# stulacy/bmm-mcmc

Hardware: AMD Instinct MI355X
Metric: gibbs_sweeps_per_s (higher is better)
Workload: dtype f64; 1 GPU; c5: gibbs_collapsed K=20 N=10000000 P=100, 1 chain per GPU; sampler=collapsed, K=20, N=10000000, P=100, batch=2500000, chains=1, chains_per_gpu=1, burn_sweeps=30, x_layout=bit planes, ceil(P/32) words per observation, packed once at hand-over

## Files before the change

bmm-mcmc_amd/csrc/chain.hip:

```cpp
#include <hip/hip_runtime.h>
#include <hip/hip_ext.h>
#include <rccl/rccl.h>

#include <dlfcn.h>
#include <emmintrin.h>
#include <sched.h>
#include <sys/mman.h>

#include <cmath>
#include <cstdarg>
#include <cstdio>
#include <cstdint>
#include <cstdlib>
#include <cstring>
#include <atomic>
#include <chrono>
#include <condition_variable>
#include <exception>
#include <functional>
#include <limits>
#include <memory>
#include <mutex>
#include <new>
#include <string>
// ... 267 lines not shown
#ifndef BMM_SMALL_SPLIT
#define BMM_SMALL_SPLIT 1
#endif
#ifndef BMM_SELF_TABLES
#define BMM_SELF_TABLES 1
#endif
constexpr int kStageWide = BMM_STAGE_WIDE;

constexpr int threads_for(int kt, bool bits) {
    if (bits) return kt <= 20 ? kThreadsSmall : (kt <= 32 ? kThreadsMid : kThreadsLarge);
    return kt <= 12 ? kThreadsSmall : (kt <= 20 ? kThreadsMid : kThreadsLarge);
}

struct KernelForm {
    int kt = 0;
    int nt = 0;
    int minus = 0;
    bool bits = false;
    int lanes = 1;
    bool emit = false;
    int gw = kGroupW;
    bool self = false;
    bool pk = false;
};
constexpr int tile_of(const KernelForm& f) { return f.nt / f.lanes; }
constexpr KernelForm resized(KernelForm f, int nt, int lanes = 1) { f.nt = nt; f.lanes = lanes; return f; }
constexpr KernelForm emit_twin(const KernelForm& f) {
    return KernelForm{f.kt, threads_for(f.kt, true), f.minus, true, 1, true, f.gw, false};
}

constexpr int stage_width(const KernelForm& f, bool named_size) {
    if (f.bits || f.kt > 20 || f.nt == 256) return 16;
    if (f.nt == kThreadsSmall) return f.nt == threads_for(f.kt, false) && !named_size ? kStageWide : 16;
    return kStageWide;
}

constexpr bool instantiated(const KernelForm& f, bool named_size) {
    const bool preferred = f.gw == kGroupW;
    if (f.pk) return f.bits && f.lanes == 1 && f.minus == 1 && !f.emit && !f.self && f.kt <= 32 &&
                     (preferred || (f.gw == kGroupWAlt && f.nt == threads_for(f.kt, true)));
    if (f.self) return f.kt <= 12 && f.nt == 256 && f.minus == 1 && f.bits && f.lanes == 1 && !f.emit && preferred;
    if (f.emit) return f.bits && f.lanes == 1 && f.nt == threads_for(f.kt, true);
    if (f.lanes == 2) return f.bits && f.nt == kThreadsSplit && f.minus != 2 && (f.kt > 32 || (f.kt >= 16 && preferred));
    if (f.lanes != 1) return false;
    if (f.nt == threads_for(f.kt, f.bits) && !named_size) return true;
    if (!preferred || f.minus == 2) return false;
    if (f.nt == 256) return true;
    return (f.nt == 1024 || f.nt == 768 || f.nt == 512) && f.kt <= 32 && (f.bits || f.minus == 1);
}

typedef void (*resample_fn)(ChainParams, ResampleArgs);
template <int KT, int NT, int MINUS, bool BITS, int GW, int LANES, bool EMIT, bool SELF, bool NAMED>
resample_fn instance() {
    constexpr KernelForm F{KT, NT, MINUS, BITS, LANES, EMIT, GW, SELF};
    if constexpr (instantiated(F, NAMED)) return k_resample<KT, NT, MINUS, stage_width(F, NAMED), BITS, LANES, EMIT, GW, SELF>;
    else return nullptr;
}
resample_fn lookup(const KernelForm& f, bool named_size = false) {
    resample_fn fn = nullptr;
    if (f.pk) {
        if (!instantiated(f, named_size)) return nullptr;
        lift([&](auto kt, auto nt, auto gw) {
            if constexpr (instantiated(KernelForm{kt, nt, 1, true, 1, false, gw, false, true}, false)) fn = k_resample_pk<kt, nt, gw>;
        }, kKT, f.kt, IntList<1024, 768, 512, 256>{}, f.nt, IntList<kGroupW, kGroupWAlt>{}, f.gw);
        return fn;
    }
    lift([&](auto kt, auto nt, auto minus, auto bits, auto gw) {
        if (f.lanes == 2) fn = f.emit || f.self ? nullptr : instance<kt, nt, minus, bits != 0, gw, 2, false, false, false>();
        else if (f.lanes != 1 || (f.emit && f.self)) fn = nullptr;
        else if (f.emit) fn = instance<kt, nt, minus, bits != 0, gw, 1, true, false, false>();
        else if (f.self) fn = instance<kt, nt, minus, bits != 0, gw, 1, false, true, false>();
        else if (named_size) fn = instance<kt, nt, minus, bits != 0, gw, 1, false, false, true>();
        else fn = instance<kt, nt, minus, bits != 0, gw, 1, false, false, false>();
    }, kKT, f.kt, IntList<1024, 768, 512, 256>{}, f.nt, IntList<0, 1, 2>{}, f.minus, IntList<0, 1>{}, (int)f.bits,
       IntList<kGroupW, kGroupWAlt>{}, f.gw);
    return fn;
}

constexpr int kLooMaxOwnKT = 32;
typedef void (*score_fn)(ChainParams, ScoreArgs);
score_fn lookup_score(int kt, int gw, int minus, bool loo) {
    score_fn fn = nullptr;
    lift([&](auto KT, auto GW, auto MINUS) {
        if constexpr (MINUS == 0) fn = loo ? k_score<KT, kScoreThreads, GW, 0, true> : k_score<KT, kScoreThreads, GW, 0, false>;
        else if constexpr (KT <= kLooMaxOwnKT) fn = loo ? k_score<KT, kScoreThreads, GW, MINUS, true> : nullptr;
    }, kKT, kt, IntList<kGroupW, kGroupWAlt>{}, gw, IntList<0, 1, 2>{}, minus);
// ... 283 lines not shown

constexpr int64_t kLargeN = (int64_t)1 << 16;
int64_t default_batch(int sampler, int64_t N) {
    if (sampler == BMM_SAMPLER_SB || sampler == BMM_SAMPLER_FULL) return N;
    const int64_t div = N >= kLargeN ? 4 : (sampler == BMM_SAMPLER_DP ? 16 : 8);
    const int64_t b = N / div;
    return b < 1 ? 1 : b;
}

TableLayout layout_of(const bmm_chain* c) { return layout_of(c->p, !explicit_params(c->p.mode)); }

int dbg_env_int(const char* name, int unset) { const char* v = dbg_env(name); return v ? (atoi(v) > 0 ? atoi(v) : 0) : unset; }
struct DebugSwitches {
    bool generic = dbg_env("BMM_DEBUG_GENERIC");
    bool int32_layout = dbg_env("BMM_X_LAYOUT_INT32");
    int cus = dbg_env_int("BMM_DEBUG_CUS", 0);
    int threads = dbg_env_int("BMM_DEBUG_THREADS", -1);
    bool split = dbg_env("BMM_DEBUG_SPLIT");
    bool nosplit = dbg_env("BMM_DEBUG_NOSPLIT");
    bool small = dbg_env("BMM_DEBUG_SMALL");
    bool noself = dbg_env("BMM_DEBUG_NOSELF");
    bool nopk = dbg_env("BMM_DEBUG_NOPK");
    bool pk = dbg_env("BMM_DEBUG_PK");
    int pk_defer_every = dbg_env_int("BMM_DEBUG_PK_DEFER_EVERY", 0);
};

struct ChainShape {
    ChainParams p{};
    int64_t batch = 1;
    bool generic = false;
    int minus_in_lds = 1;
    size_t lds_bytes_base = 0;
};
ChainParams geometry(int sampler, int P, int K, int kt, int W) {
    ChainParams q{};
    q.mode = sampler; q.P = P; q.K = K; q.KT = kt; q.W = W;
    q.G = (P + W - 1) / W; q.Gm = (P + kGroupWm - 1) / kGroupWm;
    q.Kc = sampler == BMM_SAMPLER_DP ? K + 1 : K;
    return q;
}
size_t image_bytes(const ChainParams& q, bool own_tables) {
    const TableLayout l = layout_of(q, own_tables && !explicit_params(q.mode));
    return (size_t)(own_tables ? l.doubles() : l.head()) * sizeof(double) + ((size_t)q.K * q.P + q.K + 4) * sizeof(int32_t);
}

size_t pk_image_bytes(const ChainParams& q) {
// ... 141 lines not shown
        const size_t off = (used + 255) & ~(size_t)255;
        used = off + n * sizeof(T);
        return base ? reinterpret_cast<T*>(base + off) : nullptr;
    }
};

int chain_alloc(bmm_chain* c) {
    const ChainParams& p = c->p;
    HIP_TRY(hipSetDevice(c->device));
    {
        int rcs = chain_stream_create(c, false);
        if (rcs) return rcs;
    }
    const size_t nz = (size_t)p.N;
    const size_t ns = (size_t)p.K * p.P, nn = (size_t)p.K;
    const size_t ntab = (size_t)layout_of(c).doubles() + (explicit_params(p.mode) ? 0 : 2 * (size_t)pk_tq_doubles(layout_of(c)));
    auto carve = [&](Carver& a) {
        c->dNk = a.take<int32_t>(nn);
        c->dDNk = a.take<int32_t>(nn * kDeltaReps);
        c->dS = a.take<int32_t>(ns);
        c->dDS = a.take<int32_t>(ns * kDeltaReps);
        c->dTab = a.take<double>(ntab);
#ifdef BMM_DIAG
        c->dDiag = a.take<unsigned long long>(16);
#endif
        c->dSelfDone = a.take<int>(1);
        c->dViable = a.take<int>(1);
        c->dDNkAlt = a.take<int32_t>(nn * kDeltaReps);
        c->dDSAlt = a.take<int32_t>(ns * kDeltaReps);
#ifdef BMM_DEBUG_HOOKS
        c->dDbgFlag = a.take<int>(1);
        c->dPkStat = a.take<unsigned long long>(3);
#endif
        const size_t zeroed = a.used;
        c->dAlpha = a.take<double>(1);
        c->dPi = a.take<double>(nn);
        c->dTheta = a.take<double>(ns);
        c->dZ[0] = a.take<int32_t>(nz);
        c->dZ[1] = a.take<int32_t>(nz);
        return zeroed;
    };
    Carver measure{nullptr};
    carve(measure);
    c->arena = static_cast<char*>(dev_pool().get(c->device, measure.used, &c->arena_bytes));
    if (!c->arena) return set_err(BMM_E_HIP, "allocating the chain's state failed: %s", hipGetErrorString(hipGetLastError()));
    Carver real{c->arena};
    const size_t zeroed = carve(real);
// ... 635 lines not shown
    if (c->fs_on) {
        const int rc = enqueue_fs_gamma(c, j);
        if (rc) return rc;
    }
    const int rc = sweep_end_folds(c, j);
    return rc == BMM_OK && c->na_on ? enqueue_na_step(c, j) : rc;
}

struct KernelPlan {
    int n = 0;
    KernelForm form[3];
    size_t lds[3] = {0, 0, 0};
    bool named_size = false;
};
KernelPlan plan_kernel(const ChainParams& p, bool bits, int minus, int64_t batch, int num_cus, bool shares_device,
                       size_t lds_bytes_base, const DebugSwitches& d, bool masked = false) {
    const bool alt = p.W != kGroupW;
    KernelForm f{p.KT, threads_for(p.KT, bits), minus, bits, 1, false, p.W, false};
    KernelPlan plan;
    const size_t pk_lds = explicit_params(p.mode) ? 0 : pk_image_bytes(p);
    auto offer = [&](KernelForm g, size_t lds) {
        KernelForm h = g;
        h.pk = true;
#ifdef BMM_EXP_PK_ALWAYS
        const bool long_launch = true;
#else
        const bool long_launch = batch >= (int64_t)4 * num_cus * g.nt;
#endif
        if (!masked && !d.nopk && (long_launch || d.pk) && !g.self && !explicit_params(p.mode) && instantiated(h, false) &&
            pk_lds <= kLdsMax && batch < ((int64_t)1 << 31)) { g = h; lds = pk_lds; }
        plan.form[plan.n] = g; plan.lds[plan.n++] = lds;
    };
    const bool short_launch = BMM_SMALL_SPLIT && !shares_device && p.KT >= 16 && !alt && (batch < (int64_t)num_cus * kThreadsMid || d.split);
    if (bits && (p.KT > 32 || short_launch) && minus != 2 && !d.nosplit) {
        const KernelForm g = resized(f, kThreadsSplit, 2);
        if (instantiated(g, false)) f = g;
    }
    if (d.threads >= 0 && !alt) {
        const KernelForm g = resized(f, d.threads);
        if (instantiated(g, true) && (p.KT <= 20 || (bits && g.nt != 1024))) { f = g; plan.named_size = true; }
    } else if (bits && f.lanes == 1 && !alt) {
        for (int nt : {768, 512}) {
            if ((batch + f.nt - 1) / f.nt >= num_cus || nt >= f.nt || (batch + nt - 1) / nt > num_cus) continue;
            if (instantiated(resized(f, nt), false)) f = resized(f, nt);
        }
    }
// ... 186 lines not shown
    c->minus_in_lds = shape.minus_in_lds;
    c->lds_bytes_base = c->lds_bytes = shape.lds_bytes_base;
    if (c->generic) {
        c->form = KernelForm{p.KT, 256, tier_of(c), c->bits, 1, false, p.W, false};
        c->scratch_stride = generic_threads(p.Kc);
        c->grid_max = (int)(c->scratch_stride / 256);
    } else {
        c->num_cus = dbg.cus >= 1 ? dbg.cus : cus;
        rc = pick_kernel(c);
        if (rc) { delete c; return rc; }
    }
    rc = chain_alloc(c);
    if (rc) { bmm_chain_destroy(c); return rc; }
    *out = c;
    return BMM_OK;
}

void bmm_chain_destroy(bmm_chain* c) {
    if (!c) return;
    (void)hipSetDevice(c->device);
    if (c->stream) (void)hipStreamSynchronize(c->stream);
#ifdef BMM_DIAG
    if (c->dDiag) {
        unsigned long long d[16] = {};
        const bool ok = hipMemcpy(d, c->dDiag, sizeof d, hipMemcpyDeviceToHost) == hipSuccess;
        if (ok && d[5] && d[0]) {
            const double tot = (double)(d[0] + d[1] + d[2] + d[3] + d[4]);
            fprintf(stderr, "[bmm diag] waves=%llu cycles/wave: score %.0f (%.1f%%) pack %.0f (%.1f%%) draw %.0f (%.1f%%) movers %.0f (%.1f%%) prologue %.0f (%.1f%%) movers/wave-launch %.2f\n",
                    d[5], d[0] / (double)d[5], 100 * d[0] / tot, d[1] / (double)d[5], 100 * d[1] / tot, d[2] / (double)d[5],
                    100 * d[2] / tot, d[3] / (double)d[5], 100 * d[3] / tot, d[4] / (double)d[5], 100 * d[4] / tot, d[6] / (double)d[5]);
        }
        if (ok && d[5])
            fprintf(stderr, "[bmm diag launch] ticks per wave and launch: table staging %.0f, tile loop %.0f, waiting for the workgroup %.0f, flush %.0f\n",
                    d[8] / (double)d[5], d[9] / (double)d[5], d[10] / (double)d[5], d[11] / (double)d[5]);
        if (ok && d[7])
            fprintf(stderr, "[bmm diag launch pk] workgroup-launches %llu, ticks from entry to flushed %.0f\n", d[7], d[14] / (double)d[7]);
        if (ok && d[5] && d[12])
            fprintf(stderr, "[bmm diag draw] draws of a wave (64 observations) %llu, of them by the binary64 definition %llu (%.4f%%)\n",
                    d[12], d[13], 100.0 * (double)d[13] / (double)d[12]);
    }
#endif
    for (hipEvent_t e : c->ev) (void)hipEventDestroy(e);
    if (c->planes && c->planes->refs.fetch_sub(1) == 1) {
        dev_pool().put(c->device, c->planes->d, c->planes->bytes);
        delete c->planes;
    }
    dev_pool().put(c->device, c->arena, c->arena_bytes);
    dev_pool().put(c->device, c->run_arena, c->run_arena_bytes);
    void* bufs[] = {c->dX_owned, c->dScratch, c->dProbs, c->dWts, c->dWtot, c->dXnb, c->dPredTab, c->dPredMax, c->dPredSum, c->dRespAcc,
                    c->dLooTab, c->dLooAcc, c->dLooOut, c->dLooScratch, c->dSmSide, c->dSmSideLaunch, c->dSmLq, c->dSmStat, c->dSmCell,
                    c->dSmCounters, c->dFsBlock, c->dEaBlock, c->dEaSide, c->dAsBlock, c->dLjBlock, c->dLjZ, c->dPcFeat, c->dPcXt, c->dPcBlock, c->dNaBlock};
    for (void* b : bufs)
        if (b) (void)hipFree(b);
    chain_stream_release(c->device, c->stream, c->stream_kind);
    delete c;
}

static int pack_rows(bmm_chain* c, const int32_t* dX, int64_t rows, int64_t ldx, int64_t i0) {
    const int64_t nb = (rows + 255) / 256;
// ... 3431 lines not shown
        HostCrew crew;
        crew.run(N, 1024, 64, [&](int64_t lo, int64_t hi) {
            seen.fetch_or(pack_rows_host(X, N, P, lo, hi, plane.data(), 0), std::memory_order_relaxed);
        });
        *seen_out = seen.load();
        return BMM_OK;
    });
}
extern "C" int bmm_dbg_host_labels(const void* src, int narrow, int32_t* dst, int64_t n, int jobs) {
    return guarded([&]() -> int {
        HostCrew crew;
        for (int j = 0; j < jobs; ++j) {
            if (narrow) crew.run(n, 256, 64, [=](int64_t lo, int64_t hi) { widen_labels(static_cast<const uint8_t*>(src) + lo, dst + lo, hi - lo); });
            else crew.run(n, 256, 64, [=](int64_t lo, int64_t hi) { copy_labels(static_cast<const int32_t*>(src) + lo, dst + lo, hi - lo); });
        }
        return BMM_OK;
    });
}
static void kernel_key(const KernelForm& f, const KernelForm& twin, bool generic, int grid_max_emit, int* key) {
    const int k[10] = {f.kt, f.nt, f.lanes, f.minus, f.bits ? 1 : 0, f.gw, f.self ? 1 : 0, generic ? 0 : twin.nt, generic ? 1 : 0, grid_max_emit};
    std::memcpy(key, k, sizeof k);
}
extern "C" int bmm_dbg_kernel_packed(const bmm_chain* c) { return c && !c->generic && c->form.pk ? 1 : 0; }
extern "C" int bmm_dbg_pk_counts(bmm_chain* c, unsigned long long* draws, unsigned long long* deferred) {
    if (!c || !draws || !deferred) return set_err(BMM_E_ARG, "null argument");
    return guarded([&]() -> int {
        unsigned long long v[2] = {0, 0};
        HIP_TRY(hipSetDevice(c->device));
        HIP_TRY(hipStreamSynchronize(c->stream));
        HIP_TRY(hipMemcpy(v, c->dPkStat, sizeof v, hipMemcpyDeviceToHost));
        *draws = v[0]; *deferred = v[1];
        return BMM_OK;
    });
}
extern "C" int bmm_dbg_pk_unselected(bmm_chain* c, unsigned long long* n) {
    if (!c || !n) return set_err(BMM_E_ARG, "null argument");
    return guarded([&]() -> int {
        HIP_TRY(hipSetDevice(c->device));
        HIP_TRY(hipStreamSynchronize(c->stream));
        HIP_TRY(hipMemcpy(n, c->dPkStat + 2, sizeof *n, hipMemcpyDeviceToHost));
        return BMM_OK;
    });
}
extern "C" int bmm_dbg_kernel_key(const bmm_chain* c, int* key) {
    if (!c || !key) return set_err(BMM_E_ARG, "null argument");
    kernel_key(c->form, c->form_emit, c->generic, c->fn_emit ? c->grid_max_emit : 0, key);
// ... 983 lines not shown
```

bmm-mcmc_amd/csrc/kernels.hip.h:

```cpp
#pragma once
#include <hip/hip_runtime.h>
#include <stdint.h>

#include "bmm_spec.h"

namespace bmm {

typedef __attribute__((address_space(3))) double lds_f64;

constexpr int kMaxP = 128;
constexpr int lcm_(int a, int b) { int x = a; while (x % b) x += a; return x; }
constexpr int kChunkP = kMaxP / lcm_(lcm_(kGroupW, kGroupWAlt), kGroupWm) * lcm_(lcm_(kGroupW, kGroupWAlt), kGroupWm);
constexpr int kMaxCats = 64;
constexpr int kMaxCatsAny = 1024;

enum : int { MODE_COLLAPSED = 0, MODE_DP = 1, MODE_SB = 2, MODE_FULL = 3 };
__host__ __device__ inline bool explicit_params(int mode) { return mode == MODE_SB || mode == MODE_FULL; }

struct TableLayout {
    int G, KT, Gm, M;
    __host__ __device__ int tp() const { return 0; }
    __host__ __device__ int cp() const { return G * KT * M; }
    __host__ __device__ int cm() const { return cp() + KT; }
    __host__ __device__ int nk() const { return cm() + KT; }
// ... 1053 lines not shown
        int zn = new_label;
        if (own_single && (zn < 0 || zo < zn)) zn = zo;
        return zn;
    }
    int best = -1, bs = 0;
    for (int k = 0; k < K; ++k) {
        const int sz = NkT[k] - (k == zo ? 1 : 0);
        if (sz > 0 && (best < 0 || sz < bs)) { best = k; bs = sz; }
    }
    return best >= 0 ? best : zoc;
}
__device__ __forceinline__ unsigned pk_field(int bit, unsigned mask, uint32_t b0, uint32_t b1, uint32_t b2, uint32_t b3) {
    const int wd = bit >> 5;
    return __builtin_amdgcn_alignbit(word_of(wd + 1, b0, b1, b2, b3), word_of(wd, b0, b1, b2, b3), (unsigned)(bit & 31)) & mask;
}

__device__ __forceinline__ double pk_bcast(double x, int j) {
    const long long b = __double_as_longlong(x);
    const uint64_t e = (uint64_t)(uint32_t)__builtin_amdgcn_readlane((int)(uint32_t)b, j) |
                       ((uint64_t)(uint32_t)__builtin_amdgcn_readlane((int)(uint32_t)(b >> 32), j) << 32);
    return __longlong_as_double((long long)e);
}

template <int KT, int GW>
__device__ __forceinline__ int pk_exact_count(const ChainParams& p, const ResampleArgs& a, const TableLayout& L,
                                              uint32_t w0, uint32_t w1, uint32_t w2, uint32_t w3, int zo, double u,
                                              const lds_f64* ET, int lane) {
    constexpr int GM = 1 << GW;
    constexpr int GR = KT <= 4 ? 6 : KT <= 8 ? 10 : 20;
    static_assert((kMaxP + GW - 1) / GW <= 64, "lane g holds the field of group g");
    const int G = p.G;
    const int zoc = zo < 0 ? 0 : zo;
    const int k = lane < KT ? lane : KT - 1;
    const double* const tp = a.tab + L.tp();
    const int gmp = L.gm_pad();
    const int go = lane < gmp ? lane : gmp - 1;
    const double oe = a.tab[L.tm() + ((size_t)go * KT + zoc) * kGroupMm + pk_field(go * kGroupWm, kGroupMm - 1, w0, w1, w2, w3)];
    const unsigned koff = (unsigned)k * GM;
    const int gl = lane < G ? lane : G - 1;
    const int fld = (int)pk_field(gl * GW, GM - 1, w0, w1, w2, w3);
    double sc = 0.0;
#pragma unroll 1
    for (int g0 = 0; g0 < G; g0 += GR) {
        double tv[GR];
#pragma unroll
        for (int v = 0; v < GR; ++v) {
            const int g = g0 + v < G ? g0 + v : G - 1;
            const double* const row = tp + ((size_t)g * KT * GM + (unsigned)__builtin_amdgcn_readlane(fld, g));
            tv[v] = row[koff];
        }
#pragma unroll
        for (int v = 0; v < GR; ++v)
// ... 55 lines not shown
};
__device__ __forceinline__ PkPos pk_pos(uint32_t n, int chunk, int lane) {
    PkPos t;
    t.s0 = (uint32_t)chunk << 6;
    const uint32_t room = n - 1u - t.s0;
    t.valid = (uint32_t)lane <= room;
    t.loff = (uint32_t)lane < room ? (uint32_t)lane : room;
    return t;
}
template <class T>
__device__ __forceinline__ T* pk_at(T* sbase, uint32_t loff) {
    static_assert(sizeof(T) == 4, "words and labels");
    return (T*)((const char*)sbase + (loff * 4u));
}
__device__ __forceinline__ void pk_load_words(const uint32_t* Xb, int64_t N, int W, const PkPos& t, uint32_t& w0,
                                              uint32_t& w1, uint32_t& w2, uint32_t& w3) {
    const uint32_t* const b = Xb + t.s0;
    w0 = *pk_at(b, t.loff);
    if (W > 1) w1 = *pk_at(b + N, t.loff);
    if (W > 2) w2 = *pk_at(b + 2 * N, t.loff);
    if (W > 3) w3 = *pk_at(b + 3 * N, t.loff);
}

template <int KT>
__device__ __forceinline__ bool pk_draw2(const pk_f2 (&s2)[KT / 2], float m, double u, int G, float unit, int& cnt) {
    static_assert(KT % 2 == 0 && KT <= kTier1MaxCats, "the band is derived for at most kTier1MaxCats categories");
    constexpr int KP = KT / 2;
    const pk_f2 mm{m, m}, l2e{0x1.715476p+0f, 0x1.715476p+0f};
    pk_f2 c[KP];
    float run = 0.0f;
#pragma unroll
    for (int j = 0; j < KP; ++j) {
        const pk_f2 x = (s2[j] - mm) * l2e;
        run = run + __builtin_amdgcn_exp2f(x.x);
        c[j].x = run;
        run = run + __builtin_amdgcn_exp2f(x.y);
        c[j].y = run;
    }
    const float t = (float)u * run;
    const pk_f2 tt{t, t};
    float nearest = __builtin_inff();
    int n = 0;
#pragma unroll
    for (int j = 0; j < KP; ++j) {
        const pk_f2 diff = tt - c[j];
        n += diff.x >= 0.0f ? 1 : 0;
        nearest = __builtin_fminf(nearest, __builtin_fabsf(diff.x));
        n += diff.y >= 0.0f ? 1 : 0;
        nearest = __builtin_fminf(nearest, __builtin_fabsf(diff.y));
    }
    cnt = n;
    return nearest > pk_band(m, G, unit) * run && m > -__builtin_inff() && m < __builtin_inff();
}
__device__ __forceinline__ double pk_uniform(uint64_t seed, uint64_t i0, uint32_t s0, uint32_t loff, uint32_t sweep,
                                             bool key_uniform) {
    uint32_t ra, rb;
    if (key_uniform) {
        uint32_t k = z_key(seed, 0);
        asm volatile("" : "+s"(k));
        philox2x32_10((uint32_t)i0 + s0 + loff, sweep, k, ra, rb);
        asm volatile("" : "+v"(ra), "+v"(rb));
    } else {
        const uint64_t i = i0 + s0 + loff;
        philox2x32_10((uint32_t)i, sweep, z_key(seed, i), ra, rb);
    }
    return u52(ra, rb);
}

template <int KT, int NT, int GW>
__global__ __launch_bounds__(NT) void k_resample_pk(ChainParams p, ResampleArgs a) {
    static_assert(KT % 2 == 0 && KT <= 32, "pairs of categories, one lane per category in pk_exact_count");
    constexpr int GM = 1 << GW;
    constexpr int KP = KT / 2;
    constexpr int CH = KP <= 12 ? KP : KP / 2;
    static_assert(KP % CH == 0, "chunking");
    constexpr int NW = NT / 64;
    extern __shared__ __attribute__((aligned(16))) char smem[];
    const TableLayout L{p.G, KT, p.Gm, GM};
    double* const lds = reinterpret_cast<double*>(smem);
    const int nq_d = pk_tq_doubles(L), tail_d = L.tm() - L.nk();
    const volatile lds_pk_f2* const Tq = (const volatile lds_pk_f2*)lds;
    const volatile lds_f32* const Tm32 = (const volatile lds_f32*)(lds + nq_d);
    double* const tail = lds + 2 * nq_d;
    int32_t* const hist = reinterpret_cast<int32_t*>(tail + tail_d);
    const int P = p.P, G = p.G, K = p.K;
    const int tid = threadIdx.x, lane = tid & 63;
    int* const next_chunk = hist + K * P + K;
    DIAG(const unsigned long long d_entry = diag_stamp();)
    const uint32_t n = (uint32_t)(a.hi - a.lo);
    const int nchunks = (int)((n + 63u) >> 6);
    const int cpw = (nchunks + (int)gridDim.x - 1) / (int)gridDim.x;
    const int wg_c0 = (int)blockIdx.x * cpw;
// ... 9 lines not shown
            const double2* src = reinterpret_cast<const double2*>(from);
            double2* dst = reinterpret_cast<double2*>(to);
            for (int i0 = tid; i0 < n2; i0 += NT * 8) {
                double2 t[8];
#pragma unroll
                for (int u = 0; u < 8; ++u) {
                    const int i = i0 + u * NT;
                    t[u] = src[i < n2 ? i : n2 - 1];
                }
#pragma unroll
                for (int u = 0; u < 8; ++u) {
                    const int i = i0 + u * NT;
                    if (i < n2) dst[i] = t[u];
                }
            }
        };
        stage(a.tab + L.doubles(), lds, nq_d);
        stage(a.tab + L.nk(), tail, tail_d / 2);
    }
    for (int i = tid; i < K * P + K; i += NT) hist[i] = 0;
    if (tid == 0) *next_chunk = NW;
    __syncthreads();
    DIAG(const unsigned long long d_staged = diag_stamp();)

    float unit = kPkEpsUnit;
#ifdef BMM_DEBUG_HOOKS
    if (a.dbg_inject & 8) unit = 0.0f;
    unsigned ndeferred = 0, nunselected = 0;
#endif

    if (has_tile) {
        const uint32_t* const Xb = a.Xb;
        const int32_t* const z_in = a.z_in;
        int32_t* const z_out = a.z_out;
        const int64_t N = p.N;
        const uint64_t seed = p.seed, i0 = (uint64_t)(p.obs0 + a.lo);
        const uint32_t sweep = a.sweep;
        int key_general = (int)(uint32_t)(((uint64_t)(p.obs0 + a.hi) - 1u) >> 32);
#ifdef BMM_DEBUG_HOOKS
        if (a.dbg_inject & 16) key_general = 1;
#endif
        key_general = __builtin_amdgcn_readfirstlane(key_general);
        const int dp_K = p.mode == MODE_DP ? K : -1;
        const int has_zin = (int)((uint32_t)((uintptr_t)z_in >> 32) | (uint32_t)(uintptr_t)z_in);
        int zo = -1;
        if (z_in) zo = *pk_at(z_in + pos.s0, pos.loff);
        asm volatile("" : "+v"(zo));
        int zn_prev = 0;
        uint32_t st_s0 = 0, st_loff = 0;
        bool st_on = false;
        for (;;) {
            const int zoc = zo < 0 ? 0 : zo;
            if (st_on) *pk_at(z_out + st_s0, st_loff) = zn_prev;
            int nc = 0;
            if (lane == 0) nc = atomicAdd(next_chunk, 1);
            nc = __builtin_amdgcn_readfirstlane(nc);
            const bool has_next = nc < wg_cn;
            const PkPos npos = pk_pos(n, has_next ? wg_c0 + nc : 0, lane);
            uint32_t n0 = 0, n1 = 0, n2 = 0, n3 = 0;
            int zo_next = -1;
            int Wl = W, zl = has_zin;
            asm volatile("" : "+s"(Wl), "+s"(zl));

            pk_f2 acc[KP];
#pragma unroll
            for (int j = 0; j < KP; ++j) acc[j] = pk_f2{0.0f, 0.0f};
            float own32 = 0.0f;
            const volatile lds_f32* const orow0 = Tm32 + zoc * GM;
            __builtin_amdgcn_s_setprio(BMM_LOOKUP_PRIO);
#pragma unroll 1
            for (int h = 0; h < W; ++h) {
                if (has_next && h == 0) {
                    pk_load_words(Xb, N, Wl, npos, n0, n1, n2, n3);
                    if (zl) zo_next = *pk_at(z_in + npos.s0, npos.loff);
                }
                const uint32_t cur = word_of(h, b0, b1, b2, b3), nxt = word_of(h + 1, b0, b1, b2, b3);
                const int g_lo = (32 * h + GW - 1) / GW;
                int g_hi = (32 * (h + 1) + GW - 1) / GW;
                g_hi = g_hi < G ? g_hi : G;
#pragma unroll 1
                for (int g = g_lo; g < g_hi; ++g) {
                    const unsigned nib = __builtin_amdgcn_alignbit(nxt, cur, (unsigned)(g * GW - 32 * h)) & (unsigned)(GM - 1);
                    const volatile lds_pk_f2* row = Tq + ((size_t)g * KP * GM + nib);
                    const volatile lds_f32* orow = orow0 + ((size_t)g * KT * GM + nib);
#pragma unroll
                    for (int c0 = 0; c0 < KP; c0 += CH) {
                        pk_f2 tv[CH];
                        float ov = 0.0f;
#pragma unroll
                        for (int j = 0; j < CH; ++j) tv[j] = row[(c0 + j) * GM];
                        if (c0 == 0) ov = *orow;
#pragma unroll
                        for (int j = 0; j < CH; ++j) acc[c0 + j] = acc[c0 + j] + tv[j];
                        if (c0 == 0) own32 = own32 + ov;
                        if (CH < KP) __builtin_amdgcn_sched_barrier(0);
                    }
                }
            }
            __builtin_amdgcn_s_setprio(0);
            pk_f2 s2[KP];
            float m = -__builtin_inff();
#pragma unroll
            for (int j = 0; j < KP; ++j) {
                float x = acc[j].x, y = acc[j].y;
                if (2 * j == zo) x = own32;
                if (2 * j + 1 == zo) y = own32;
                s2[j] = pk_f2{x, y};
                m = __builtin_fmaxf(m, x);
                m = __builtin_fmaxf(m, y);
            }
            int kg = key_general;
            asm volatile("" : "+s"(kg));
            const double u = pk_uniform(seed, i0, pos.s0, pos.loff, sweep, kg == 0);
            int cnt = 0;
            bool certain = pk_draw2<KT>(s2, m, u, G, unit, cnt);
            DBG_TIER1_FORCE(a, certain);
            bool defer = pos.valid && !certain;
#ifdef BMM_DEBUG_HOOKS
            const bool selected = a.pk_defer_every > 0 && pos.valid &&
                                  (a.lo + (int64_t)pos.s0 + lane) % a.pk_defer_every == 0;
            nunselected += (unsigned)__popcll(__ballot(defer && !selected));
            defer = defer || selected;
#endif
            int zn = cnt;
            unsigned long long o = __ballot(defer);
#ifdef BMM_DEBUG_HOOKS
            ndeferred += (unsigned)__popcll(o);
#endif
            if (__builtin_expect(o != 0, 0)) {
                const PkArgsView v = pk_args_view();
                const TableLayout Lc{v.p->G, KT, v.p->Gm, GM};
                const PkLds lc = pk_lds(smem, Lc);
                int ln = lane;
                asm volatile("" : "+v"(ln));
                do {
                    const int src = __ffsll((long long)o) - 1;
                    o &= o - 1;
                    const uint32_t w0 = __builtin_amdgcn_readlane(b0, src), w1 = __builtin_amdgcn_readlane(b1, src);
                    const uint32_t w2 = __builtin_amdgcn_readlane(b2, src), w3 = __builtin_amdgcn_readlane(b3, src);
                    const int e = pk_exact_count<KT, GW>(*v.p, *v.a, Lc, w0, w1, w2, w3, __builtin_amdgcn_readlane(zo, src),
                                                         pk_bcast(u, src), lc.ET, ln);
                    if (ln == src) zn = e;
                } while (o);
            }
            if (__builtin_expect(__ballot(zn == dp_K) != 0, 0)) {
                const PkArgsView v = pk_args_view();
                const int Kc = v.p->K;
                const TableLayout Lc{v.p->G, KT, v.p->Gm, GM};
                const int32_t* const Nkc = pk_lds(smem, Lc).NkT;
                int Kused = 0, new_label = -1;
                for (int k = 0; k < Kc; ++k) {
                    if (Nkc[k] > 0) ++Kused;
                    else if (new_label < 0) new_label = k;
                }
                if (zn == Kc) zn = pk_dp_label(Nkc, Kc, Kused, new_label, zo, zoc);
            }
            const bool keep = pos.valid;
#ifdef BMM_DEBUG_HOOKS
            BMM_DBG_LABELS(a, keep, pos.s0 + (uint32_t)lane == 0u, K, zn, zo);
#endif
            const bool moves = keep && zn >= 0 && zn != zo;
            if (__builtin_expect(__ballot(moves) != 0, 0)) {
                const PkArgsView v = pk_args_view();
                const int Kc = v.p->K, Pc = v.p->P;
                const TableLayout Lc{v.p->G, KT, v.p->Gm, GM};
                int ln = lane;
                asm volatile("" : "+v"(ln));
                count_movers(moves, zo, zn, b0, b1, b2, b3, pk_lds(smem, Lc).hist, Kc, Pc, ln);
            }
            zn_prev = zn;
            st_s0 = pos.s0; st_loff = pos.loff; st_on = keep;
            if (!has_next) break;
            b0 = n0; b1 = n1; b2 = n2; b3 = n3;
            zo = zo_next;
            pos = npos;
        }
        if (st_on) *pk_at(z_out + st_s0, st_loff) = zn_prev;
    }

    DIAG(const unsigned long long d_loop = diag_stamp();)
    __syncthreads();
    DIAG(const unsigned long long d_sync = diag_stamp();)
    {
        const PkArgsView v = pk_args_view();
        const int Kc = v.p->K, Pc = v.p->P;
        const TableLayout Lc{v.p->G, KT, v.p->Gm, GM};
        const int rep = blockIdx.x % kDeltaReps;
        flush_hist(pk_lds(smem, Lc).hist, Kc, Pc, v.a->dS + (size_t)rep * Kc * Pc, v.a->dNk + rep * Kc, tid, NT);
    }
    DIAG(asm volatile("s_waitcnt vmcnt(0)" ::: "memory"); const unsigned long long d_flush = diag_stamp();)
    DIAG(if (a.diag && tid == 0) {
        atomicAdd(&a.diag[5], 1ull); atomicAdd(&a.diag[7], 1ull); atomicAdd(&a.diag[14], d_flush - d_entry);
        atomicAdd(&a.diag[8], d_staged - d_entry); atomicAdd(&a.diag[9], d_loop - d_staged);
        atomicAdd(&a.diag[10], d_sync - d_loop); atomicAdd(&a.diag[11], d_flush - d_sync);
    })
#ifdef BMM_DEBUG_HOOKS
    if (a.pk_stat) {
        if (tid == 0) {
            int64_t first = a.lo + (int64_t)wg_c0 * 64, last = a.lo + ((int64_t)wg_c0 + (wg_cn > 0 ? wg_cn : 0)) * 64;
            last = last < a.hi ? last : a.hi;
            if (last > first) atomicAdd(&a.pk_stat[0], (unsigned long long)(last - first));
        }
        if (lane == 0 && ndeferred) atomicAdd(&a.pk_stat[1], (unsigned long long)ndeferred);
        if (lane == 0 && nunselected) atomicAdd(&a.pk_stat[2], (unsigned long long)nunselected);
    }
#endif
}

__device__ __forceinline__ unsigned field_from_x(const int32_t* X, const uint32_t* Xb, int64_t N, int P,
                                                  int64_t i, int g, int GW) {
    if (Xb) {
        const int o = g * GW, w = o >> 5, sh = o & 31, W = (P + 31) >> 5;
        uint32_t v = Xb[(int64_t)w * N + i] >> sh;
        if (sh + GW > 32 && w + 1 < W) v |= Xb[(int64_t)(w + 1) * N + i] << (32 - sh);
        return v & (unsigned)((1 << GW) - 1);
    }
    unsigned nib = 0;
// ... 2768 lines not shown
```

Baseline: 3560 sweeps/s.

## Software-pipeline packed resample: overlap previous draw with next observation's table lookups

Adds a pipelined variant of the packed resample kernel, used for 1024-thread blocks with at most 20 categories. It interleaves the exp/cumulative-sum and compare phases of the previous observation's categorical draw into the per-group LDS table-lookup rounds of the current observation. The goal is to hide the draw's ALU latency behind LDS loads. It also caps the exact-count fallback's group rounds at 10 in this path and adds diagnostics counters, at the cost of more registers and more code complexity.

```diff
diff --git a/bmm-mcmc_amd/csrc/chain.hip b/bmm-mcmc_amd/csrc/chain.hip
--- a/bmm-mcmc_amd/csrc/chain.hip
+++ b/bmm-mcmc_amd/csrc/chain.hip
@@ -313,6 +313,7 @@
     int gw = kGroupW;
     bool self = false;
     bool pk = false;
+    bool pipe = false;
 };
 constexpr int tile_of(const KernelForm& f) { return f.nt / f.lanes; }
 constexpr KernelForm resized(KernelForm f, int nt, int lanes = 1) { f.nt = nt; f.lanes = lanes; return f; }
@@ -350,9 +351,12 @@
 resample_fn lookup(const KernelForm& f, bool named_size = false) {
     resample_fn fn = nullptr;
     if (f.pk) {
-        if (!instantiated(f, named_size)) return nullptr;
+        if (!instantiated(f, named_size) || (f.pipe && !pk_pipelined(f.kt, f.nt, f.gw))) return nullptr;
         lift([&](auto kt, auto nt, auto gw) {
-            if constexpr (instantiated(KernelForm{kt, nt, 1, true, 1, false, gw, false, true}, false)) fn = k_resample_pk<kt, nt, gw>;
+            if constexpr (instantiated(KernelForm{kt, nt, 1, true, 1, false, gw, false, true}, false)) {
+                fn = k_resample_pk<kt, nt, gw, false>;
+                if constexpr (pk_pipelined(kt, nt, gw)) if (f.pipe) fn = k_resample_pk<kt, nt, gw, true>;
+            }
         }, kKT, f.kt, IntList<1024, 768, 512, 256>{}, f.nt, IntList<kGroupW, kGroupWAlt>{}, f.gw);
         return fn;
     }
@@ -682,6 +686,7 @@
     bool noself = dbg_env("BMM_DEBUG_NOSELF");
     bool nopk = dbg_env("BMM_DEBUG_NOPK");
     bool pk = dbg_env("BMM_DEBUG_PK");
+    bool nopipe = dbg_env("BMM_DEBUG_PK_NOPIPE");
     int pk_defer_every = dbg_env_int("BMM_DEBUG_PK_DEFER_EVERY", 0);
 };
 
@@ -869,7 +874,7 @@
         c->dDS = a.take<int32_t>(ns * kDeltaReps);
         c->dTab = a.take<double>(ntab);
 #ifdef BMM_DIAG
-        c->dDiag = a.take<unsigned long long>(16);
+        c->dDiag = a.take<unsigned long long>(18);
 #endif
         c->dSelfDone = a.take<int>(1);
         c->dViable = a.take<int>(1);
@@ -1551,6 +1556,7 @@
     auto offer = [&](KernelForm g, size_t lds) {
         KernelForm h = g;
         h.pk = true;
+        h.pipe = pk_pipelined(h.kt, h.nt, h.gw) && !d.nopipe;
 #ifdef BMM_EXP_PK_ALWAYS
         const bool long_launch = true;
 #else
@@ -1783,7 +1789,7 @@
     if (c->stream) (void)hipStreamSynchronize(c->stream);
 #ifdef BMM_DIAG
     if (c->dDiag) {
-        unsigned long long d[16] = {};
+        unsigned long long d[18] = {};
         const bool ok = hipMemcpy(d, c->dDiag, sizeof d, hipMemcpyDeviceToHost) == hipSuccess;
         if (ok && d[5] && d[0]) {
             const double tot = (double)(d[0] + d[1] + d[2] + d[3] + d[4]);
@@ -1796,6 +1802,9 @@
                     d[8] / (double)d[5], d[9] / (double)d[5], d[10] / (double)d[5], d[11] / (double)d[5]);
         if (ok && d[7])
             fprintf(stderr, "[bmm diag launch pk] workgroup-launches %llu, ticks from entry to flushed %.0f\n", d[7], d[14] / (double)d[7]);
+        if (ok && d[7] && d[17])
+            fprintf(stderr, "[bmm diag trip pk] trips of wave 0: %llu, ticks per trip: scoring %.0f, outside it %.0f\n", d[17],
+                    d[16] / (double)d[17], ((double)d[9] - (double)d[16]) / (double)d[17]);
         if (ok && d[5] && d[12])
             fprintf(stderr, "[bmm diag draw] draws of a wave (64 observations) %llu, of them by the binary64 definition %llu (%.4f%%)\n",
                     d[12], d[13], 100.0 * (double)d[13] / (double)d[12]);
@@ -5273,6 +5282,7 @@
     std::memcpy(key, k, sizeof k);
 }
 extern "C" int bmm_dbg_kernel_packed(const bmm_chain* c) { return c && !c->generic && c->form.pk ? 1 : 0; }
+extern "C" int bmm_dbg_kernel_pk_pipelined(const bmm_chain* c) { return c && !c->generic && c->form.pk && c->form.pipe ? 1 : 0; }
 extern "C" int bmm_dbg_pk_counts(bmm_chain* c, unsigned long long* draws, unsigned long long* deferred) {
     if (!c || !draws || !deferred) return set_err(BMM_E_ARG, "null argument");
     return guarded([&]() -> int {
diff --git a/bmm-mcmc_amd/csrc/kernels.hip.h b/bmm-mcmc_amd/csrc/kernels.hip.h
--- a/bmm-mcmc_amd/csrc/kernels.hip.h
+++ b/bmm-mcmc_amd/csrc/kernels.hip.h
@@ -1099,12 +1099,12 @@
     return __longlong_as_double((long long)e);
 }
 
-template <int KT, int GW>
+template <int KT, int GW, int GRMAX = 20>
 __device__ __forceinline__ int pk_exact_count(const ChainParams& p, const ResampleArgs& a, const TableLayout& L,
                                               uint32_t w0, uint32_t w1, uint32_t w2, uint32_t w3, int zo, double u,
                                               const lds_f64* ET, int lane) {
     constexpr int GM = 1 << GW;
-    constexpr int GR = KT <= 4 ? 6 : KT <= 8 ? 10 : 20;
+    constexpr int GR0 = KT <= 4 ? 6 : KT <= 8 ? 10 : 20, GR = GR0 < GRMAX ? GR0 : GRMAX;
     static_assert((kMaxP + GW - 1) / GW <= 64, "lane g holds the field of group g");
     const int G = p.G;
     const int zoc = zo < 0 ? 0 : zo;
@@ -1206,33 +1206,38 @@
     if (W > 3) w3 = *pk_at(b + 3 * N, t.loff);
 }
 
+__device__ __forceinline__ void pk_exp_slice(pk_f2& sc, float m, float& run) {
+    const pk_f2 mm{m, m}, l2e{0x1.715476p+0f, 0x1.715476p+0f};
+    const pk_f2 x = (sc - mm) * l2e;
+    run = run + __builtin_amdgcn_exp2f(x.x);
+    sc.x = run;
+    run = run + __builtin_amdgcn_exp2f(x.y);
+    sc.y = run;
+}
+__device__ __forceinline__ void pk_cmp_slice(const pk_f2& c, float t, int& n, float& nearest) {
+    const pk_f2 tt{t, t};
+    const pk_f2 diff = tt - c;
+    n += diff.x >= 0.0f ? 1 : 0;
+    nearest = __builtin_fminf(nearest, __builtin_fabsf(diff.x));
+    n += diff.y >= 0.0f ? 1 : 0;
+    nearest = __builtin_fminf(nearest, __builtin_fabsf(diff.y));
+}
 template <int KT>
 __device__ __forceinline__ bool pk_draw2(const pk_f2 (&s2)[KT / 2], float m, double u, int G, float unit, int& cnt) {
     static_assert(KT % 2 == 0 && KT <= kTier1MaxCats, "the band is derived for at most kTier1MaxCats categories");
     constexpr int KP = KT / 2;
-    const pk_f2 mm{m, m}, l2e{0x1.715476p+0f, 0x1.715476p+0f};
     pk_f2 c[KP];
     float run = 0.0f;
 #pragma unroll
     for (int j = 0; j < KP; ++j) {
-        const pk_f2 x = (s2[j] - mm) * l2e;
-        run = run + __builtin_amdgcn_exp2f(x.x);
-        c[j].x = run;
-        run = run + __builtin_amdgcn_exp2f(x.y);
-        c[j].y = run;
+        c[j] = s2[j];
+        pk_exp_slice(c[j], m, run);
     }
     const float t = (float)u * run;
-    const pk_f2 tt{t, t};
     float nearest = __builtin_inff();
     int n = 0;
 #pragma unroll
-    for (int j = 0; j < KP; ++j) {
-        const pk_f2 diff = tt - c[j];
-        n += diff.x >= 0.0f ? 1 : 0;
-        nearest = __builtin_fminf(nearest, __builtin_fabsf(diff.x));
-        n += diff.y >= 0.0f ? 1 : 0;
-        nearest = __builtin_fminf(nearest, __builtin_fabsf(diff.y));
-    }
+    for (int j = 0; j < KP; ++j) pk_cmp_slice(c[j], t, n, nearest);
     cnt = n;
     return nearest > pk_band(m, G, unit) * run && m > -__builtin_inff() && m < __builtin_inff();
 }
@@ -1251,7 +1256,201 @@
     return u52(ra, rb);
 }
 
-template <int KT, int NT, int GW>
+template <int I>
+struct PkIdx { static constexpr int value = I; };
+template <int I, int N, class F>
+__device__ __forceinline__ void pk_static_for(F&& f) {
+    if constexpr (I < N) {
+        f(PkIdx<I>{});
+        pk_static_for<I + 1, N>(f);
+    }
+}
+template <int KT, int GW, int g, class Fill>
+__device__ __forceinline__ void pk_step(const volatile lds_pk_f2* Tq, const volatile lds_f32* orow0, uint32_t b0,
+                                        uint32_t b1, uint32_t b2, uint32_t b3, pk_f2 (&acc)[KT / 2], float& own32,
+                                        Fill&& fill) {
+    constexpr int GM = 1 << GW, KP = KT / 2, CH = KP <= 12 ? KP : KP / 2;
+    constexpr int bit = g * GW, wd = bit >> 5, sh = bit & 31;
+    static_assert(bit < kMaxP, "a group of the pattern");
+    const uint32_t lo = wd == 0 ? b0 : (wd == 1 ? b1 : (wd == 2 ? b2 : b3));
+    const uint32_t hi = wd == 0 ? b1 : (wd == 1 ? b2 : (wd == 2 ? b3 : 0u));
+    const unsigned nib = (sh + GW <= 32 ? lo >> sh : __builtin_amdgcn_alignbit(hi, lo, (unsigned)sh)) & (unsigned)(GM - 1);
+    const volatile lds_pk_f2* row = Tq + ((size_t)g * KP * GM + nib);
+    const volatile lds_f32* orow = orow0 + ((size_t)g * KT * GM + nib);
+#pragma unroll
+    for (int c0 = 0; c0 < KP; c0 += CH) {
+        pk_f2 tv[CH];
+        float ov = 0.0f;
+#pragma unroll
+        for (int j = 0; j < CH; ++j) tv[j] = row[(c0 + j) * GM];
+        if (c0 == 0) ov = *orow;
+        if (c0 == 0) fill();
+#pragma unroll
+        for (int j = 0; j < CH; ++j) acc[c0 + j] = acc[c0 + j] + tv[j];
+        if (c0 == 0) own32 = own32 + ov;
+        if (CH < KP) __builtin_amdgcn_sched_barrier(0);
+    }
+}
+
+#define BMM_PK_PIN2(a, i) "+v"(a[i]), "+v"(a[(i) + 1])
+template <int KT>
+__device__ __forceinline__ void pk_step_end(pk_f2 (&acc)[KT / 2]) {
+    constexpr int KP = KT / 2;
+    static_assert(KP % 2 == 0 && KP <= 16, "pairs of sums");
+    if constexpr (KP == 2) asm volatile("" : BMM_PK_PIN2(acc, 0));
+    if constexpr (KP == 4) asm volatile("" : BMM_PK_PIN2(acc, 0), BMM_PK_PIN2(acc, 2));
+    if constexpr (KP == 6) asm volatile("" : BMM_PK_PIN2(acc, 0), BMM_PK_PIN2(acc, 2), BMM_PK_PIN2(acc, 4));
+    if constexpr (KP >= 8) asm volatile("" : BMM_PK_PIN2(acc, 0), BMM_PK_PIN2(acc, 2), BMM_PK_PIN2(acc, 4), BMM_PK_PIN2(acc, 6));
+    if constexpr (KP == 10) asm volatile("" : BMM_PK_PIN2(acc, 8));
+    if constexpr (KP == 12) asm volatile("" : BMM_PK_PIN2(acc, 8), BMM_PK_PIN2(acc, 10));
+    if constexpr (KP == 14) asm volatile("" : BMM_PK_PIN2(acc, 8), BMM_PK_PIN2(acc, 10), BMM_PK_PIN2(acc, 12));
+    if constexpr (KP == 16) asm volatile("" : BMM_PK_PIN2(acc, 8), BMM_PK_PIN2(acc, 10), BMM_PK_PIN2(acc, 12), BMM_PK_PIN2(acc, 14));
+    __builtin_amdgcn_sched_barrier(0);
+}
+#undef BMM_PK_PIN2
+template <int KT, int GW>
+__device__ __forceinline__ void pk_groups(const volatile lds_pk_f2* Tq, const volatile lds_f32* orow0, int g_from, int g_to,
+                                          int W, uint32_t b0, uint32_t b1, uint32_t b2, uint32_t b3, pk_f2 (&acc)[KT / 2],
+                                          float& own32) {
+    constexpr int GM = 1 << GW, KP = KT / 2, CH = KP <= 12 ? KP : KP / 2;
+#pragma unroll 1
+    for (int h = (g_from * GW) >> 5; h < W; ++h) {
+        const uint32_t cur = word_of(h, b0, b1, b2, b3), nxt = word_of(h + 1, b0, b1, b2, b3);
+        int g_lo = (32 * h + GW - 1) / GW;
+        g_lo = g_lo > g_from ? g_lo : g_from;
+        int g_hi = (32 * (h + 1) + GW - 1) / GW;
+        g_hi = g_hi < g_to ? g_hi : g_to;
+#pragma unroll 1
+        for (int g = g_lo; g < g_hi; ++g) {
+            const unsigned nib = __builtin_amdgcn_alignbit(nxt, cur, (unsigned)(g * GW - 32 * h)) & (unsigned)(GM - 1);
+            const volatile lds_pk_f2* row = Tq + ((size_t)g * KP * GM + nib);
+            const volatile lds_f32* orow = orow0 + ((size_t)g * KT * GM + nib);
+#pragma unroll
+            for (int c0 = 0; c0 < KP; c0 += CH) {
+                pk_f2 tv[CH];
+                float ov = 0.0f;
+#pragma unroll
+                for (int j = 0; j < CH; ++j) tv[j] = row[(c0 + j) * GM];
+                if (c0 == 0) ov = *orow;
+#pragma unroll
+                for (int j = 0; j < CH; ++j) acc[c0 + j] = acc[c0 + j] + tv[j];
+                if (c0 == 0) own32 = own32 + ov;
+                if (CH < KP) __builtin_amdgcn_sched_barrier(0);
+            }
+        }
+    }
+}
+template <int KT, int GW, bool DRAW, class Head>
+__device__ __forceinline__ void pk_rounds(const volatile lds_pk_f2* Tq, const volatile lds_f32* orow0, int G, int W,
+                                          uint32_t b0, uint32_t b1, uint32_t b2, uint32_t b3, pk_f2 (&acc)[KT / 2],
+                                          float& own32, pk_f2 (&c)[KT / 2], float m, const double& u, float& run, int& cnt,
+                                          float& nearest, Head&& head) {
+    constexpr int KP = KT / 2;
+    constexpr bool kRound0 = (KP - 1) * GW < kMaxP, kRound1 = (2 * KP - 1) * GW < kMaxP;
+    asm volatile("" : "+s"(G));
+    bool whole = false;
+    if constexpr (kRound0) whole = G >= KP;
+    if (whole) {
+        if constexpr (kRound0)
+            pk_static_for<0, KP>([&](auto J) {
+                constexpr int j = decltype(J)::value;
+                pk_step<KT, GW, j>(Tq, orow0, b0, b1, b2, b3, acc, own32, [&] {
+                    if constexpr (j == 0) head();
+                    if constexpr (DRAW) pk_exp_slice(c[j], m, run);
+                });
+                pk_step_end<KT>(acc);
+            });
+    } else {
+        head();
+        pk_groups<KT, GW>(Tq, orow0, 0, G < KP ? G : KP, W, b0, b1, b2, b3, acc, own32);
+        if constexpr (DRAW) pk_static_for<0, KP>([&](auto J) { pk_exp_slice(c[decltype(J)::value], m, run); });
+    }
+    float t = 0.0f;
+    if constexpr (DRAW) t = (float)u * run;
+    whole = false;
+    if constexpr (kRound1) whole = G >= 2 * KP;
+    if (whole) {
+        if constexpr (kRound1)
+            pk_static_for<0, KP>([&](auto J) {
+                constexpr int j = decltype(J)::value;
+                pk_step<KT, GW, KP + j>(Tq, orow0, b0, b1, b2, b3, acc, own32, [&] {
+                    if constexpr (DRAW) pk_cmp_slice(c[j], t, cnt, nearest);
+                });
+                pk_step_end<KT>(acc);
+            });
+        if (G > 2 * KP) pk_groups<KT, GW>(Tq, orow0, 2 * KP, G, W, b0, b1, b2, b3, acc, own32);
+    } else {
+        if (G > KP) pk_groups<KT, GW>(Tq, orow0, KP, G, W, b0, b1, b2, b3, acc, own32);
+        if constexpr (DRAW) pk_static_for<0, KP>([&](auto J) { pk_cmp_slice(c[decltype(J)::value], t, cnt, nearest); });
+    }
+}
+
+constexpr bool pk_pipelined(int kt, int nt, int ) { return nt == 1024 && kt <= 20; }
+
+template <int KT, int GW, int GRMAX = 20>
+__device__ __forceinline__ int pk_settle(const ResampleArgs& a, char* smem, const PkPos& pos, int lane, bool certain,
+                                         int cnt, double u, int zo, uint32_t b0, uint32_t b1, uint32_t b2, uint32_t b3,
+                                         int dp_K, int K, unsigned& ndeferred, unsigned& nunselected) {
+    constexpr int GM = 1 << GW;
+    const int zoc = zo < 0 ? 0 : zo;
+    DBG_TIER1_FORCE(a, certain);
+    bool defer = pos.valid && !certain;
+#ifdef BMM_DEBUG_HOOKS
+    const bool selected = a.pk_defer_every > 0 && pos.valid &&
+                          (a.lo + (int64_t)pos.s0 + lane) % a.pk_defer_every == 0;
+    nunselected += (unsigned)__popcll(__ballot(defer && !selected));
+    defer = defer || selected;
+#endif
+    int zn = cnt;
+    unsigned long long o = __ballot(defer);
+#ifdef BMM_DEBUG_HOOKS
+    ndeferred += (unsigned)__popcll(o);
+#endif
+    if (__builtin_expect(o != 0, 0)) {
+        const PkArgsView v = pk_args_view();
+        const TableLayout Lc{v.p->G, KT, v.p->Gm, GM};
+        const PkLds lc = pk_lds(smem, Lc);
+        int ln = lane;
+        asm volatile("" : "+v"(ln));
+        do {
+            const int src = __ffsll((long long)o) - 1;
+            o &= o - 1;
+            const uint32_t w0 = __builtin_amdgcn_readlane(b0, src), w1 = __builtin_amdgcn_readlane(b1, src);
+            const uint32_t w2 = __builtin_amdgcn_readlane(b2, src), w3 = __builtin_amdgcn_readlane(b3, src);
+            const int e = pk_exact_count<KT, GW, GRMAX>(*v.p, *v.a, Lc, w0, w1, w2, w3, __builtin_amdgcn_readlane(zo, src),
+                                                        pk_bcast(u, src), lc.ET, ln);
+            if (ln == src) zn = e;
+        } while (o);
+    }
+    if (__builtin_expect(__ballot(zn == dp_K) != 0, 0)) {
+        const PkArgsView v = pk_args_view();
+        const int Kc = v.p->K;
+        const TableLayout Lc{v.p->G, KT, v.p->Gm, GM};
+        const int32_t* const Nkc = pk_lds(smem, Lc).NkT;
+        int Kused = 0, new_label = -1;
+        for (int k = 0; k < Kc; ++k) {
+            if (Nkc[k] > 0) ++Kused;
+            else if (new_label < 0) new_label = k;
+        }
+        if (zn == Kc) zn = pk_dp_label(Nkc, Kc, Kused, new_label, zo, zoc);
+    }
+    const bool keep = pos.valid;
+#ifdef BMM_DEBUG_HOOKS
+    BMM_DBG_LABELS(a, keep, pos.s0 + (uint32_t)lane == 0u, K, zn, zo);
+#endif
+    const bool moves = keep && zn >= 0 && zn != zo;
+    if (__builtin_expect(__ballot(moves) != 0, 0)) {
+        const PkArgsView v = pk_args_view();
+        const int Kc = v.p->K, Pc = v.p->P;
+        const TableLayout Lc{v.p->G, KT, v.p->Gm, GM};
+        int ln = lane;
+        asm volatile("" : "+v"(ln));
+        count_movers(moves, zo, zn, b0, b1, b2, b3, pk_lds(smem, Lc).hist, Kc, Pc, ln);
+    }
+    return zn;
+}
+
+template <int KT, int NT, int GW, bool PIPE>
 __global__ __launch_bounds__(NT) void k_resample_pk(ChainParams p, ResampleArgs a) {
     static_assert(KT % 2 == 0 && KT <= 32, "pairs of categories, one lane per category in pk_exact_count");
     constexpr int GM = 1 << GW;
@@ -1307,12 +1506,13 @@
     if (tid == 0) *next_chunk = NW;
     __syncthreads();
     DIAG(const unsigned long long d_staged = diag_stamp();)
+    DIAG(unsigned long long d_score = 0, d_trips = 0;)
 
     float unit = kPkEpsUnit;
 #ifdef BMM_DEBUG_HOOKS
     if (a.dbg_inject & 8) unit = 0.0f;
+#endif
     unsigned ndeferred = 0, nunselected = 0;
-#endif
 
     if (has_tile) {
         const uint32_t* const Xb = a.Xb;
@@ -1331,6 +1531,7 @@
         int zo = -1;
         if (z_in) zo = *pk_at(z_in + pos.s0, pos.loff);
         asm volatile("" : "+v"(zo));
+        if constexpr (!PIPE) {
         int zn_prev = 0;
         uint32_t st_s0 = 0, st_loff = 0;
         bool st_on = false;
@@ -1352,6 +1553,7 @@
             for (int j = 0; j < KP; ++j) acc[j] = pk_f2{0.0f, 0.0f};
             float own32 = 0.0f;
             const volatile lds_f32* const orow0 = Tm32 + zoc * GM;
+            DIAG(const unsigned long long d_s0 = diag_stamp();)
             __builtin_amdgcn_s_setprio(BMM_LOOKUP_PRIO);
 #pragma unroll 1
             for (int h = 0; h < W; ++h) {
@@ -1383,6 +1585,7 @@
                 }
             }
             __builtin_amdgcn_s_setprio(0);
+            DIAG(d_score += diag_stamp() - d_s0; ++d_trips;)
             pk_f2 s2[KP];
             float m = -__builtin_inff();
 #pragma unroll
@@ -1398,61 +1601,10 @@
             asm volatile("" : "+s"(kg));
             const double u = pk_uniform(seed, i0, pos.s0, pos.loff, sweep, kg == 0);
             int cnt = 0;
-            bool certain = pk_draw2<KT>(s2, m, u, G, unit, cnt);
-            DBG_TIER1_FORCE(a, certain);
-            bool defer = pos.valid && !certain;
-#ifdef BMM_DEBUG_HOOKS
-            const bool selected = a.pk_defer_every > 0 && pos.valid &&
-                                  (a.lo + (int64_t)pos.s0 + lane) % a.pk_defer_every == 0;
-            nunselected += (unsigned)__popcll(__ballot(defer && !selected));
-            defer = defer || selected;
-#endif
-            int zn = cnt;
-            unsigned long long o = __ballot(defer);
-#ifdef BMM_DEBUG_HOOKS
-            ndeferred += (unsigned)__popcll(o);
-#endif
-            if (__builtin_expect(o != 0, 0)) {
-                const PkArgsView v = pk_args_view();
-                const TableLayout Lc{v.p->G, KT, v.p->Gm, GM};
-                const PkLds lc = pk_lds(smem, Lc);
-                int ln = lane;
-                asm volatile("" : "+v"(ln));
-                do {
-                    const int src = __ffsll((long long)o) - 1;
-                    o &= o - 1;
-                    const uint32_t w0 = __builtin_amdgcn_readlane(b0, src), w1 = __builtin_amdgcn_readlane(b1, src);
-                    const uint32_t w2 = __builtin_amdgcn_readlane(b2, src), w3 = __builtin_amdgcn_readlane(b3, src);
-                    const int e = pk_exact_count<KT, GW>(*v.p, *v.a, Lc, w0, w1, w2, w3, __builtin_amdgcn_readlane(zo, src),
-                                                         pk_bcast(u, src), lc.ET, ln);
-                    if (ln == src) zn = e;
-                } while (o);
-            }
-            if (__builtin_expect(__ballot(zn == dp_K) != 0, 0)) {
-                const PkArgsView v = pk_args_view();
-                const int Kc = v.p->K;
-                const TableLayout Lc{v.p->G, KT, v.p->Gm, GM};
-                const int32_t* const Nkc = pk_lds(smem, Lc).NkT;
-                int Kused = 0, new_label = -1;
-                for (int k = 0; k < Kc; ++k) {
-                    if (Nkc[k] > 0) ++Kused;
-                    else if (new_label < 0) new_label = k;
-                }
-                if (zn == Kc) zn = pk_dp_label(Nkc, Kc, Kused, new_label, zo, zoc);
-            }
+            const bool certain = pk_draw2<KT>(s2, m, u, G, unit, cnt);
+            const int zn = pk_settle<KT, GW>(a, smem, pos, lane, certain, cnt, u, zo, b0, b1, b2, b3, dp_K, K, ndeferred,
+                                             nunselected);
             const bool keep = pos.valid;
-#ifdef BMM_DEBUG_HOOKS
-            BMM_DBG_LABELS(a, keep, pos.s0 + (uint32_t)lane == 0u, K, zn, zo);
-#endif
-            const bool moves = keep && zn >= 0 && zn != zo;
-            if (__builtin_expect(__ballot(moves) != 0, 0)) {
-                const PkArgsView v = pk_args_view();
-                const int Kc = v.p->K, Pc = v.p->P;
-                const TableLayout Lc{v.p->G, KT, v.p->Gm, GM};
-                int ln = lane;
-                asm volatile("" : "+v"(ln));
-                count_movers(moves, zo, zn, b0, b1, b2, b3, pk_lds(smem, Lc).hist, Kc, Pc, ln);
-            }
             zn_prev = zn;
             st_s0 = pos.s0; st_loff = pos.loff; st_on = keep;
             if (!has_next) break;
@@ -1461,6 +1613,104 @@
             pos = npos;
         }
         if (st_on) *pk_at(z_out + st_s0, st_loff) = zn_prev;
+        } else {
+        pk_f2 s2[KP];
+#pragma unroll
+        for (int j = 0; j < KP; ++j) s2[j] = pk_f2{0.0f, 0.0f};
+        float pm = 0.0f;
+        PkPos ppos;
+        ppos.s0 = pos.s0; ppos.loff = pos.loff; ppos.valid = pos.valid;
+        int pzo = -1;
+        uint32_t q0 = 0, q1 = 0, q2 = 0, q3 = 0;
+        bool have_prev = false, have_cur = true;
+        for (;;) {
+            bool certain = false, has_next = false;
+            int cnt = 0;
+            double u = 0.0;
+            PkPos npos;
+            npos.s0 = pos.s0; npos.loff = pos.loff; npos.valid = pos.valid;
+            uint32_t n0 = 0, n1 = 0, n2 = 0, n3 = 0;
+            int zo_next = -1;
+            pk_f2 acc[KP];
+#pragma unroll
+            for (int j = 0; j < KP; ++j) acc[j] = pk_f2{0.0f, 0.0f};
+            float own32 = 0.0f;
+            int kg = key_general;
+            asm volatile("" : "+s"(kg));
+            if (have_cur) {
+                const int zoc = zo < 0 ? 0 : zo;
+                int nc = 0;
+                if (lane == 0) nc = atomicAdd(next_chunk, 1);
+                int Wl = W, zl = has_zin;
+                asm volatile("" : "+s"(Wl), "+s"(zl));
+                const volatile lds_f32* const orow0 = Tm32 + zoc * GM;
+                auto grab = [&] {
+                    __builtin_amdgcn_sched_barrier(0);
+                    nc = __builtin_amdgcn_readfirstlane(nc);
+                    has_next = nc < wg_cn;
+                    const PkPos t = pk_pos(n, has_next ? wg_c0 + nc : 0, lane);
+                    npos.s0 = t.s0; npos.loff = t.loff; npos.valid = t.valid;
+                    if (has_next) {
+                        pk_load_words(Xb, N, Wl, npos, n0, n1, n2, n3);
+                        if (zl) zo_next = *pk_at(z_in + npos.s0, npos.loff);
+                    }
+                };
+                DIAG(const unsigned long long d_s0 = diag_stamp();)
+                __builtin_amdgcn_s_setprio(BMM_LOOKUP_PRIO);
+#ifdef BMM_EXP_PK_NOOVERLAP
+                if (have_prev) {
+                    float run = 0.0f, nearest = 0.0f;
+                    pk_rounds<KT, GW, false>(Tq, orow0, G, W, b0, b1, b2, b3, acc, own32, s2, pm, u, run, cnt, nearest, [&] {
+                        grab();
+                        u = pk_uniform(seed, i0, ppos.s0, ppos.loff, sweep, kg == 0);
+                    });
+                    certain = pk_draw2<KT>(s2, pm, u, G, unit, cnt);
+                } else
+#endif
+                if (have_prev) {
+                    float run = 0.0f, nearest = __builtin_inff();
+                    pk_rounds<KT, GW, true>(Tq, orow0, G, W, b0, b1, b2, b3, acc, own32, s2, pm, u, run, cnt, nearest, [&] {
+                        grab();
+                        u = pk_uniform(seed, i0, ppos.s0, ppos.loff, sweep, kg == 0);
+                    });
+                    certain = nearest > pk_band(pm, G, unit) * run && pm > -__builtin_inff() && pm < __builtin_inff();
+                } else {
+                    float run = 0.0f, nearest = 0.0f;
+                    pk_rounds<KT, GW, false>(Tq, orow0, G, W, b0, b1, b2, b3, acc, own32, s2, pm, u, run, cnt, nearest, grab);
+                }
+                __builtin_amdgcn_s_setprio(0);
+                DIAG(d_score += diag_stamp() - d_s0; ++d_trips;)
+            } else {
+                u = pk_uniform(seed, i0, ppos.s0, ppos.loff, sweep, kg == 0);
+                certain = pk_draw2<KT>(s2, pm, u, G, unit, cnt);
+            }
+            int zn = 0;
+            if (have_prev)
+                zn = pk_settle<KT, GW, 10>(a, smem, ppos, lane, certain, cnt, u, pzo, q0, q1, q2, q3, dp_K, K, ndeferred,
+                                           nunselected);
+            asm volatile("" : "+v"(n0), "+v"(n1), "+v"(n2), "+v"(n3), "+v"(zo_next));
+            if (have_prev && ppos.valid) *pk_at(z_out + ppos.s0, ppos.loff) = zn;
+            if (!have_cur) break;
+            pm = -__builtin_inff();
+#pragma unroll
+            for (int j = 0; j < KP; ++j) {
+                float x = acc[j].x, y = acc[j].y;
+                if (2 * j == zo) x = own32;
+                if (2 * j + 1 == zo) y = own32;
+                s2[j] = pk_f2{x, y};
+                pm = __builtin_fmaxf(pm, x);
+                pm = __builtin_fmaxf(pm, y);
+            }
+            ppos.s0 = pos.s0; ppos.loff = pos.loff; ppos.valid = pos.valid;
+            pzo = zo;
+            q0 = b0; q1 = b1; q2 = b2; q3 = b3;
+            have_prev = true;
+            have_cur = has_next;
+            b0 = n0; b1 = n1; b2 = n2; b3 = n3;
+            zo = zo_next;
+            pos.s0 = npos.s0; pos.loff = npos.loff; pos.valid = npos.valid;
+        }
+        }
     }
 
     DIAG(const unsigned long long d_loop = diag_stamp();)
@@ -1478,6 +1728,7 @@
         atomicAdd(&a.diag[5], 1ull); atomicAdd(&a.diag[7], 1ull); atomicAdd(&a.diag[14], d_flush - d_entry);
         atomicAdd(&a.diag[8], d_staged - d_entry); atomicAdd(&a.diag[9], d_loop - d_staged);
         atomicAdd(&a.diag[10], d_sync - d_loop); atomicAdd(&a.diag[11], d_flush - d_sync);
+        atomicAdd(&a.diag[16], d_score); atomicAdd(&a.diag[17], d_trips);
     })
 #ifdef BMM_DEBUG_HOOKS
     if (a.pk_stat) {
```

New measurement: 3755 sweeps/s, median of 6. +5.5%, better.
